# michiyasunaga/qagnn

Hardware: AMD Instinct MI355X
Metric: QA-subgraphs/sec (batch x num_choice) fwd+bwd (higher is better)
Workload: dtype f32; 1 GPU; configs[1]: CSQA-shaped batch 64 questions x 5 choices = 320 subgraphs per GPU, n=200 node slots, 400..2000 edges/subgraph, 38 relations (run_qagnn__csqa.sh), 5-layer GAT d=200 H=4, QAGNN decoder fwd+bwd (LM encoder excluded: random sent_vecs), dropout 0.2, train-mode BN; subgraphs_per_gpu=320, nodes=64000, edges=396800, edges_with_self_loops=460800, graph_input=load-time int32 blobs (qagnn_graph_from_blobs), 13.3 B/edge on the wire, parallelism=single

## Files before the change

### __graft_entry__.py

```python
import os
import sys

ROOT = os.path.dirname(os.path.abspath(__file__))
if ROOT not in sys.path:
    sys.path.insert(0, ROOT)


def build():
    from qagnn_amd.build import build as build_lib
    path = build_lib(force=False)
    from qagnn_amd import _lib
    lib = _lib.load_library(path)
    assert lib.qagnn_abi_version() == _lib.ABI_VERSION
    for name in _lib.EXPORTS + _lib.EXPORTS_TN + _lib.EXPORTS_INFER + _lib.EXPORTS_LOSS + _lib.EXPORTS_EXPLAIN + _lib.EXPORTS_DEFER:
        assert hasattr(lib, name), name
    import qagnn_amd.modeling_qagnn
    import oracle.qagnn_oracle
    print(f'[build] {path} ok ({os.path.getsize(path)} bytes), {len(_lib.EXPORTS)} C-ABI symbols')


def smoke():
    import torch
    sys.path.insert(0, os.path.join(ROOT, 'tests'))
    import helpers
    from qagnn_amd import modeling_qagnn as MQ
    from qagnn_amd import ops
    assert torch.cuda.is_available(), 'smoke() needs an MI355X'
    torch.set_num_threads(min(os.cpu_count() or 1, 32))
    case = dict(shape='config1', nq=1, nc=5, n=100, n_rel=17, std=0.6, train=True, seed=3,
# ... 32 lines not shown
```

### qagnn_amd/_lib.py

```python
import ctypes as C
import functools
import os

import torch

_HERE = os.path.dirname(os.path.abspath(__file__))
LIB_PATH = os.environ.get('QAGNN_LIB') or os.path.join(_HERE, 'libqagnn_hip.so')

EXPORTS = ['qagnn_last_error', 'qagnn_abi_version', 'qagnn_graph_storage_elems', 'qagnn_graph_prep', 'qagnn_graph_prep_blocked',
           'qagnn_graph_from_blobs', 'qagnn_radam_step_f32', 'qagnn_node_prep_f32', 'qagnn_seed_epoch_advance', 'qagnn_seed_epoch_set',
           'qagnn_gemm_nn_f32', 'qagnn_gemm_nn_split_f32', 'qagnn_gemm_nn_pack_bytes', 'qagnn_gemm_nn_ws_bytes', 'qagnn_gemm_nn_split_ws_f32', 'qagnn_gemm_nn_prepack_bytes', 'qagnn_gemm_nn_prepack_f32',
           'qagnn_gemm_nn_prepack_clear', 'qagnn_gemm_tn_workspace_elems', 'qagnn_gemm_tn_f32', 'qagnn_gemm_tn2_f32', 'qagnn_gemm_tn_colsum_f32',
           'qagnn_colreduce_workspace_elems', 'qagnn_colreduce_f32', 'qagnn_bn_finalize_f32', 'qagnn_bn_stats_finalize_f32', 'qagnn_bn_relu_bwd_f32',
           'qagnn_gelu_dropout_fwd_f32', 'qagnn_gelu_dropout_bwd_f32', 'qagnn_sin_basis_f32',
           'qagnn_bn_relu_bwd_colsum_f32',
           'qagnn_pool_attn_fwd_f32', 'qagnn_pool_attn_bwd_f32', 'qagnn_head_post_fwd_f32', 'qagnn_head_post_bwd_f32', 'qagnn_add_row0_f32', 'qagnn_gather_multi_f32', 'qagnn_gather_multi_sum_f32',
           'qagnn_edge_attn_fwd_f32', 'qagnn_edge_attn_bwd_f32',
           'qagnn_hop_fwd_workspace_elems', 'qagnn_hop_bwd_workspace_elems', 'qagnn_hop_fwd_f32', 'qagnn_hop_bwd_f32',
           'qagnn_stack_fwd_f32', 'qagnn_stack_bwd_f32', 'qagnn_absmax_f32', 'qagnn_zero_words', 'qagnn_gemm_tn_h2_f32', 'qagnn_gelu_dropout_fwd_amax_f32', 'qagnn_gelu_dropout_amax_scratch_elems',
           'qagnn_timing_enable', 'qagnn_timing_read', 'qagnn_gemm_tn_h1_f32', 'qagnn_gelu_dropout_bwd_amax_f32', 'qagnn_packed_min_rows',
           'qagnn_radam_step_scaled_f32', 'qagnn_grad_norm_workspace_elems', 'qagnn_grad_norm_f32', 'qagnn_scale_multi_f32', 'qagnn_graph_prep_cap',
           'qagnn_store_gather', 'qagnn_graph_from_store']
EXPORTS_TN = ['qagnn_gemm_tn_graph_f32', 'qagnn_gemm_tn_route_query', 'qagnn_tn_work_table', 'qagnn_tn_live_tiles']
EXPORTS_INFER = ['qagnn_infer_version', 'qagnn_bn_relu_absmax_scratch_elems', 'qagnn_bn_relu_absmax_f32', 'qagnn_stack_infer_f32',
                 'qagnn_choice_eval_f32']
EXPORTS_LOSS = ['qagnn_loss_version', 'qagnn_choice_loss_f32', 'qagnn_choice_loss_bwd_f32']
EXPORTS_EXPLAIN = ['qagnn_explain_version', 'qagnn_attn_export_f32', 'qagnn_attn_trace_f32']
EXPORTS_DEFER = ['qagnn_defer_version', 'qagnn_stack_bwd_defer_elems', 'qagnn_stack_bwd_deferred_f32']
EXPORTS_ROWS = ['qagnn_rows_version', 'qagnn_row_groups_workspace_elems', 'qagnn_row_groups', 'qagnn_row_segment_sum_workspace_elems',
                'qagnn_row_segment_sum_f32', 'qagnn_rows_scatter_f32']
ROWS_CHUNK = 64
ROWS_MAX_N, ROWS_MAX_TABLE = 1 << 20, 1 << 26
DEFER_MAX_HOPS = 16
TRACE_MAX_N = 1024
LOSS_KINDS = {'cross_entropy': 0, 'margin_rank': 1}
LOSS_THREADS = 256

CLS_SLICES = 4
ABI_VERSION = 25

_i32, _i64, _f32, _u64, _vp = C.c_int32, C.c_int64, C.c_float, C.c_uint64, C.c_void_p


class qagnn_graph(C.Structure):
    _fields_ = ([(n, _i32) for n in ('N', 'E', 'Ep', 'R', 'T', 'C')] +
# ... 144 lines not shown
    lib.qagnn_explain_version.argtypes = []
    lib.qagnn_attn_export_f32.argtypes = [C.POINTER(qagnn_graph), _vp, _i64, _i32, _vp, _i64, _vp]
    lib.qagnn_attn_trace_f32.argtypes = [C.POINTER(qagnn_graph), _vp, _i64, _i32, _i32, _i32, _i32, _i32, _vp, _vp, _vp, _vp]
    lib.qagnn_defer_version.argtypes = []
    lib.qagnn_stack_bwd_defer_elems.restype = _i64
    lib.qagnn_stack_bwd_defer_elems.argtypes = [_i32, _i32, _i32, _i32]
    lib.qagnn_stack_bwd_deferred_f32.argtypes = [C.POINTER(qagnn_hop_args), _i32, _vp, _i64, _vp]
    lib.qagnn_rows_version.argtypes = []
    lib.qagnn_row_groups_workspace_elems.restype = _i64
    lib.qagnn_row_groups_workspace_elems.argtypes = [_i32]
    lib.qagnn_row_groups.argtypes = [_vp, _i32, _i64, _vp, _vp, _vp, _vp, _vp, _i64, _vp]
    lib.qagnn_row_segment_sum_workspace_elems.restype = _i64
    lib.qagnn_row_segment_sum_workspace_elems.argtypes = [_i32, _i32]
    lib.qagnn_row_segment_sum_f32.argtypes = [_vp, _i64, _i32, _vp, _vp, _vp, _i32, _vp, _i64, _i32, _vp, _i64, _vp]
    lib.qagnn_rows_scatter_f32.argtypes = [_vp, _i64, _i32, _vp, _vp, _i32, _vp, _i64, _i64, _i32, _vp]
    for name in EXPORTS + EXPORTS_TN + EXPORTS_INFER + EXPORTS_LOSS + EXPORTS_EXPLAIN + EXPORTS_DEFER + EXPORTS_ROWS:
        fn = getattr(lib, name)
        if fn.restype is C.c_int and name not in ('qagnn_abi_version',):
            fn.restype = _i32
    return lib


def _ptr(t):
    return None if t is None else t.data_ptr()


def choice_loss_bound(kind, nc, Q, max_abs=1.0, margin=0.0, weight=1.0, threads=LOSS_THREADS):
    import math
    u, v = 2.0 ** -24, 2.0 ** -53
    M, L, w = max(1.0, float(max_abs)), math.log(nc), abs(float(weight))
    S = -(-Q // threads) + math.log2(threads) + nc
    if LOSS_KINDS[kind] == 0:
        return w * M * (u * (nc + 8 + 5 * L) + v * S * (2 + L)), w / Q * u * (nc + 8 + L)
    return w * M * (3 * u + v * S) * (2 + abs(float(margin)) / M), w / Q * 2 * u


def _running_fields(running):
    if running is None:
        return None, None, None, None, 0, 0.0, 1.0
# ... 502 lines not shown
        return out

    def gemm_tn_graph(self, A1, A2, B, graph=None, pieces=3, amax=None, out=None):
        _chkp(A1, 'A1'), _chkp(A2, 'A2'), _chkp(B, 'B')
        Ka1, Ka2 = A1.size(1), A2.size(1)
        R, No = B.shape
        assert A1.size(0) == R and A2.size(0) == R and (pieces == 3 or amax is not None)
        out, ws = self._tn_out_ws(R, Ka1 + Ka2, No, out, B.device)
        am = [None, None, None] if amax is None else [t.data_ptr() for t in amax]
        rc = self.lib.qagnn_gemm_tn_graph_f32(A1.data_ptr(), _ld(A1), Ka1, A2.data_ptr(), _ld(A2), Ka2, B.data_ptr(), _ld(B), out.data_ptr(), _ld(out),
                                              R, No, am[0], am[1], am[2], pieces, C.byref(graph.c) if graph is not None else None, ws.data_ptr(),
                                              self._stream())
        self._check(rc, 'qagnn_gemm_tn_graph_f32')
        return out

    def tn_route_query(self, R, Ka1, Ka2, No):
        out = (_i32 * 4)()
        self._check(self.lib.qagnn_gemm_tn_route_query(R, Ka1, Ka2, No, C.cast(out, _vp)), 'qagnn_gemm_tn_route_query')
        return tuple(out)

    def tn_work_table(self, graph, S, chunk_tiles):
        out = torch.empty(4 + 5 * S, dtype=torch.int32, device=graph.storage.device)
        self._check(self.lib.qagnn_tn_work_table(C.byref(graph.c), S, chunk_tiles, out.data_ptr(), self._stream()), 'qagnn_tn_work_table')
        return out

    def tn_live_tiles(self, on):
        return int(self.lib.qagnn_tn_live_tiles(int(on)))

    def gemm_tn2(self, A1, A2, B, out=None):
        _chkp(A1, 'A1'), _chkp(A2, 'A2'), _chkp(B, 'B')
# ... 617 lines not shown
```

### qagnn_amd/build.py

```python
import hashlib
import os
import subprocess
import sys

HERE = os.path.dirname(os.path.abspath(__file__))
CSRC = os.path.join(HERE, 'csrc')
LIB = os.path.join(HERE, 'libqagnn_hip.so')
STAMP = LIB + '.srchash'
SOURCES = ['graph_prep.hip', 'gemm.hip', 'elementwise.hip', 'edge_attn.hip', 'pool.hip', 'hop.hip', 'optim.hip', 'gemm_split.hip', 'gemm_nn2.hip', 'gemm_dispatch.hip', 'timing.hip', 'infer.hip', 'loss.hip', 'explain.hip', 'rows.hip']
FLAGS = ['--offload-arch=gfx950', '-O3', '-std=c++17', '-fPIC', '-shared']


def hashed_files():
    headers = sorted(f for f in os.listdir(CSRC) if f.endswith('.h'))
    return [os.path.join(CSRC, s) for s in SOURCES + headers] + [os.path.join(HERE, '..', 'include', 'qagnn_hip.h'),
                                                                 os.path.join(HERE, '..', 'include', 'qagnn_hip_tn.h'),
                                                                 os.path.join(HERE, '..', 'include', 'qagnn_hip_infer.h'),
                                                                 os.path.join(HERE, '..', 'include', 'qagnn_hip_loss.h'),
                                                                 os.path.join(HERE, '..', 'include', 'qagnn_hip_explain.h'),
                                                                 os.path.join(HERE, '..', 'include', 'qagnn_hip_defer.h'),
                                                                 os.path.join(HERE, '..', 'include', 'qagnn_hip_rows.h')]


def source_hash():
    h = hashlib.sha256(' '.join(FLAGS).encode())
    for p in hashed_files():
        with open(p, 'rb') as f:
            h.update(os.path.basename(p).encode() + b'\0' + f.read() + b'\0')
    return h.hexdigest()


def up_to_date():
    if not (os.path.exists(LIB) and os.path.exists(STAMP)):
        return False
    with open(STAMP) as f:
        return f.read().strip() == source_hash()
# ... 20 lines not shown
```

### qagnn_amd/csrc/common.h

```cpp
#pragma once
#include <hip/hip_runtime.h>
#include <stdint.h>
#include <stdio.h>

#include <type_traits>

#include "../../include/qagnn_hip.h"
#include "../../include/qagnn_hip_tn.h"
#include "../../include/qagnn_hip_infer.h"

namespace qagnn {

void set_error(const char* fmt, ...);

struct NnProduct {
  const qagnn_gemm_nn_args* a;
  bool split;
  const float* B1n; int ldn1; const float* B2n; int ldn2;
  void* ws; int64_t ws_bytes;
};
enum class NnFamily { FP32, SPLIT, NN2 };
enum class NnB { IN_KERNEL, PACK, IMAGE };
struct NnRoute {
  NnFamily family;
// ... 7 lines not shown
  static int n = [] {
    int dev = 0, v = 0;
    if (hipGetDevice(&dev) != hipSuccess || hipDeviceGetAttribute(&v, hipDeviceAttributeMultiprocessorCount, dev) != hipSuccess || v <= 0) v = 256;
    return v;
  }();
  return n;
}
static inline int cdiv(int64_t a, int64_t b) { return (int)((a + b - 1) / b); }
inline void nn_grid(NnRoute& r, int M, int No, int rows_per_tile, int per_cu) {
  r.ntiles = cdiv(No, r.nt * 16) * cdiv(M, rows_per_tile);
  const int cap = (num_cus() * per_cu) & ~7;
  r.grid = r.ntiles < cap ? r.ntiles : cap;
}
NnRoute nn_route(const NnProduct& p);
bool nn_rows_packed(int64_t M);
int gemm_nn(const NnProduct& p, hipStream_t stream);
int launch_nn(const NnRoute& r, const qagnn_gemm_nn_args& a, hipStream_t stream);
int launch_nn_split(const NnRoute& r, const qagnn_gemm_nn_args& a, const float* B1n, int ldn1, const float* B2n, int ldn2, hipStream_t stream);
int launch_nn2(const NnRoute& r, const qagnn_gemm_nn_args& a, const float* B1n, int ldn1, const float* B2n, int ldn2, hipStream_t stream);
int launch_pack_b(int np, const qagnn_gemm_nn_args& a, const float* B1n, int ldn1, const float* B2n, int ldn2, void* ws, hipStream_t stream);
namespace nn2 { int walk_tiles(int K1, int K2); }
int64_t nn2_pack_bytes(int No, int K1, int K2, int np);
const void* nn2_prepack_lookup(const float* B1n, int ldn1, int K1, const float* B2n, int ldn2, int K2, int No, int np);

struct TnProduct {
  const float* A1; int lda1, Ka1;
  const float* A2; int lda2, Ka2; bool two;
  const float* B; int ldb;
  float* C; int ldc, R, No;
  const float* a_scale; const float* a_shift; const int64_t* a_rowidx; int accumulate;
  float* bsum; const int64_t* b_rowidx; int groups;
  const uint32_t* amax[3]; int np;
  float* ws;
  const qagnn_graph* g;
};
// ... 309 lines not shown
```

### qagnn_amd/csrc/gemm_dispatch.hip

```cpp
#include <stdlib.h>

#include <atomic>
#include <initializer_list>

#include "common.h"

namespace qagnn {

static int pick_nt(int No) {
  const int cands[5] = {13, 7, 8, 4, 2};
  for (int c : cands)
    if (No % (c * 16) == 0) return c;
  int best = 4;
  int64_t best_cost = INT64_MAX;
  for (int c : cands) {
    const int64_t cost = (int64_t)cdiv(No, c * 16) * c * 16;
    if (cost < best_cost) { best_cost = cost; best = c; }
  }
  return best;
}

static std::atomic<int64_t> g_pack_min_m{8192};
bool nn_rows_packed(int64_t M) { return M >= g_pack_min_m.load(std::memory_order_relaxed); }

static bool nn2_ok(const qagnn_gemm_nn_args& a, int ldn1, int ldn2) {
  const int64_t lim = (int64_t)0x7FFFFFFF;
  if (a.a_rowidx && !(a.a_rows > 0 && a.a_rows * (int64_t)a.lda1 * 4 < lim && a.K2 == 0)) return false;
  if (a.K1 % 8 != 0 || a.K2 % 8 != 0) return false;
  if ((int64_t)a.M * a.lda1 * 4 >= lim || (int64_t)a.No * ldn1 * 4 >= lim || (int64_t)a.M * a.ldc * 4 >= lim) return false;
  if (a.K2 > 0 && ((int64_t)a.M * a.lda2 * 4 >= lim || (int64_t)a.No * ldn2 * 4 >= lim)) return false;
  if (a.K2 > 0 && (a.K1 & 31) != 0 && a.K2 < 32 - (a.K1 & 31)) return false;
  if (a.a_scale && a.K1 > 256) return false;
  return true;
}
static bool nn2_staggered(int nt, const qagnn_gemm_nn_args& a) {
  return nt >= 8 && nn2::walk_tiles(a.K1, a.K2) >= 10 && (int64_t)cdiv(a.No, nt * 16) * cdiv(a.M, 256) * 10 >= num_cus() * 9;
}

NnRoute nn_route(const NnProduct& p) {
  const qagnn_gemm_nn_args& a = *p.a;
  NnRoute r = {};
  r.np = 3;
  r.affine = a.a_scale != nullptr;
  if (!p.split) {
    r.family = NnFamily::FP32;
    r.nt = pick_nt(a.No);
    r.wv = 8;
    nn_grid(r, a.M, a.No, 128, QAGNN_NN_OCC > 0 ? QAGNN_NN_OCC : 1);
    return r;
  }
  const int nt16 = cdiv(a.No, 16);
  r.nt = nt16 >= 13 ? 13 : nt16 >= 8 ? 8 : nt16 >= 7 ? 7 : nt16 >= 4 ? 4 : 2;
  for (int c : {7, 4, 2})
    if (cdiv(a.M, 128) * cdiv(a.No, r.nt * 16) < num_cus() * 3 / 2 && c < r.nt) r.nt = c;
  r.wv = 4;
  r.stats = a.colstat_part != nullptr;
  if (!nn2_ok(a, p.ldn1, p.ldn2)) {
    const int64_t lim = (int64_t)0x7FFFFFFF;
    r.family = NnFamily::SPLIT;
    r.flat = a.a_rowidx || (int64_t)a.M * a.lda1 * 4 >= lim || (int64_t)a.M * a.lda2 * 4 >= lim || (int64_t)a.No * p.ldn1 * 4 >= lim ||
             (int64_t)a.No * p.ldn2 * 4 >= lim;
    nn_grid(r, a.M, a.No, 128, 2);
    return r;
  }
  r.family = NnFamily::NN2;
  auto image = [&](int np) {
    const int64_t need = nn2_pack_bytes(a.No, a.K1, a.K2, np);
    if ((r.image = nn2_prepack_lookup(p.B1n, p.ldn1, a.K1, p.B2n, p.ldn2, a.K2, a.No, np))) r.b = NnB::IMAGE;
    else if (p.ws && nn_rows_packed(a.M) && p.ws_bytes >= need && (np == 3 || aligned16(p.ws))) { r.b = NnB::PACK; r.ws_bytes = need; }
    else return false;
    r.np = np;
    return true;
  };
  const bool scaled = nn_rows_packed(a.M) && a.a_amax1 && (a.K2 == 0 || a.a_amax2);
  if (!(scaled && image(a.pieces == 1 ? 1 : 2)) && !image(3)) r.b = NnB::IN_KERNEL;
  if (r.b != NnB::IN_KERNEL && r.np == 3 && nn2_staggered(r.nt, a)) r.wv = 8;
  nn_grid(r, a.M, a.No, r.wv * 32, r.wv == 8 ? 1 : 2);
  return r;
}

static int nn_validate(const NnProduct& p) {
  QAGNN_REQUIRE(p.a, QAGNN_EINVAL, "gemm_nn: null pointer");
  const qagnn_gemm_nn_args& a = *p.a;
  const float* B1 = p.split ? p.B1n : a.B1, *B2 = p.split ? p.B2n : a.B2;
  const int ldb1 = p.split ? p.ldn1 : a.ldb1, ldb2 = p.split ? p.ldn2 : a.ldb2, km = p.split ? 4 : 16;
  QAGNN_REQUIRE(a.A1 && B1 && a.C, QAGNN_EINVAL, "gemm_nn: null pointer");
  QAGNN_REQUIRE(a.M > 0 && a.No > 0 && a.K1 > 0, QAGNN_EINVAL, "gemm_nn: bad sizes M=%d No=%d K1=%d", a.M, a.No, a.K1);
  QAGNN_REQUIRE(a.K1 % km == 0 && a.K2 % km == 0 && a.K2 >= 0, QAGNN_EINVAL, "gemm_nn: K1=%d K2=%d must be multiples of %d", a.K1, a.K2, km);
  QAGNN_REQUIRE(a.No % 4 == 0, QAGNN_EINVAL, "gemm_nn: No=%d must be a multiple of 4", a.No);
  QAGNN_REQUIRE(a.lda1 % 4 == 0 && ldb1 % 4 == 0 && (!p.split || ldb1 >= a.K1) && aligned16(a.A1) && aligned16(B1), QAGNN_EINVAL,
                "gemm_nn: operand 1 must be 16-byte aligned with pitches multiple of 4");
  QAGNN_REQUIRE(a.K2 == 0 || (a.A2 && B2 && a.lda2 % 4 == 0 && ldb2 % 4 == 0 && (!p.split || ldb2 >= a.K2) && aligned16(a.A2) && aligned16(B2)),
                QAGNN_EINVAL, "gemm_nn: operand 2 must be 16-byte aligned with pitches multiple of 4");
  QAGNN_REQUIRE(!a.rowtab || a.rowidx, QAGNN_EINVAL, "gemm_nn: rowtab without rowidx");
  QAGNN_REQUIRE(a.ldc % 4 == 0 && aligned16(a.C) && (!a.bias || aligned16(a.bias)) && (!a.rowtab || (aligned16(a.rowtab) && a.ldt % 4 == 0)),
                QAGNN_EINVAL, "gemm_nn: C / bias / rowtab must be 16-byte aligned with pitches multiple of 4");
// ... 14 lines not shown
}

int gemm_nn(const NnProduct& p, hipStream_t stream) {
  TimedScope timed(0, stream);
  if (int rc = nn_validate(p)) return rc;
  const qagnn_gemm_nn_args& a = *p.a;
  const NnRoute r = nn_route(p);
  if (r.family == NnFamily::FP32) return launch_nn(r, a, stream);
  if (r.family == NnFamily::SPLIT) return launch_nn_split(r, a, p.B1n, p.ldn1, p.B2n, p.ldn2, stream);
  if (r.b == NnB::IN_KERNEL) return launch_nn2(r, a, p.B1n, p.ldn1, p.B2n, p.ldn2, stream);
  if (r.b == NnB::PACK) {
    QAGNN_REQUIRE(aligned16(p.ws), QAGNN_EINVAL, "gemm_nn: the pack workspace must be 16-byte aligned");
    if (int rc = launch_pack_b(r.np, a, p.B1n, p.ldn1, p.B2n, p.ldn2, p.ws, stream)) return rc;
  }
  return launch_nn2(r, a, static_cast<const float*>(r.b == NnB::PACK ? p.ws : r.image), cdiv(a.No, 16), nullptr, 0, stream);
}

static int tn_chunk_rows(int R, int blocks_per_chunk, int per_cu, int ktile, int lo) {
  const int target = num_cus() * per_cu / blocks_per_chunk;
  const int rows = cdiv(cdiv(R, target > 0 ? target : 1), ktile) * ktile, lo_k = cdiv(lo, ktile) * ktile;
  return rows > lo_k ? rows : lo_k;
}
static int tn_min_chunk(int R, bool split) { return R > 4096 ? 256 : split ? 32 : 64; }
static int64_t tn_ws_bound(int R, int Ka, int No) { return (int64_t)cdiv(R, tn_min_chunk(R, true)) * ((int64_t)Ka * No + 4 * (int64_t)No); }
constexpr int TN_WS_MIN_TILES = 28;

static int pick_tn_waves(int Ka) {
  int best = 4, best_waste = INT32_MAX;
  for (int nw = 16; nw >= 4; --nw) {
    const int bm = nw * 16, waste = cdiv(Ka, bm) * bm - Ka;
// ... 121 lines not shown

extern "C" int qagnn_gemm_nn_f32(const qagnn_gemm_nn_args* a, qagnn_stream_t stream) {
  return gemm_nn(NnProduct{a, false, nullptr, 0, nullptr, 0, nullptr, 0}, (hipStream_t)stream);
}

extern "C" int qagnn_gemm_nn_split_f32(const qagnn_gemm_nn_args* a, const float* B1n, int32_t ldn1, const float* B2n, int32_t ldn2,
                                       qagnn_stream_t stream) {
  return gemm_nn(NnProduct{a, true, B1n, ldn1, B2n, ldn2, nullptr, 0}, (hipStream_t)stream);
}

extern "C" int qagnn_gemm_nn_split_ws_f32(const qagnn_gemm_nn_args* a, const float* B1n, int32_t ldn1, const float* B2n, int32_t ldn2,
                                          void* ws, int64_t ws_bytes, qagnn_stream_t stream) {
  return gemm_nn(NnProduct{a, true, B1n, ldn1, B2n, ldn2, ws, ws_bytes}, (hipStream_t)stream);
}

extern "C" int64_t qagnn_gemm_tn_workspace_elems(int32_t R, int32_t Ka, int32_t No) { return tn_ws_bound(R, Ka, No); }

extern "C" int qagnn_gemm_tn_colsum_f32(const float* A, int32_t lda, const float* B, int32_t ldb, float* C, int32_t ldc, int32_t R,
                                        int32_t Ka, int32_t No, const float* a_scale, const float* a_shift, const int64_t* a_rowidx,
                                        int32_t accumulate, float* bsum, const int64_t* b_rowidx, int32_t groups, float* workspace,
                                        qagnn_stream_t stream) {
  TnProduct p = tn_product(A, lda, Ka, nullptr, 0, 0, B, ldb, C, ldc, R, No, a_scale, a_shift, workspace);
  p.a_rowidx = a_rowidx; p.accumulate = accumulate; p.bsum = bsum; p.b_rowidx = b_rowidx; p.groups = groups;
  return gemm_tn(p, (hipStream_t)stream);
}

extern "C" int qagnn_gemm_tn_f32(const float* A, int32_t lda, const float* B, int32_t ldb, float* C, int32_t ldc, int32_t R,
                                 int32_t Ka, int32_t No, const float* a_scale, const float* a_shift, const int64_t* a_rowidx,
                                 int32_t accumulate, float* workspace, qagnn_stream_t stream) {
  TnProduct p = tn_product(A, lda, Ka, nullptr, 0, 0, B, ldb, C, ldc, R, No, a_scale, a_shift, workspace);
// ... 53 lines not shown
```

### qagnn_amd/csrc/gemm_nn2.hip

```cpp
#include <stdlib.h>


#include "gemm_device.h"

namespace qagnn {

namespace nn2 {

constexpr int BK = 32;

template <bool AFFINE, int NP = 2>
__device__ __forceinline__ void split_frag2(const u32x4s (&r)[2], u32x4s (&f)[NP], const float* __restrict__ sc, const float* __restrict__ sh, float lo,
                                            float s) {
  uint32_t ph[4], pl[4];
#pragma unroll
  for (int e = 0; e < 8; e += 2) {
    const uint32_t ux = r[e >> 2][e & 3], uy = r[(e + 1) >> 2][(e + 1) & 3];
    float x = __builtin_bit_cast(float, ux), y = __builtin_bit_cast(float, uy);
    if constexpr (AFFINE) {
      x = floor_nan(fmaf(x, sc[e], sh[e]), lo);
      y = floor_nan(fmaf(y, sc[e + 1], sh[e + 1]), lo);
    }
    if constexpr (NP == 2) split2(x, y, s, ph[e >> 1], pl[e >> 1]);
    else split1(x, y, s, ph[e >> 1]);
// ... 446 lines not shown
      __syncthreads();
      QAGNN_NN_SLAB_FILL(acc[i], (lane >> 4) * 4)
      __syncthreads();
      if constexpr (STATS) {
        const float* const S0 = reinterpret_cast<const float*>(smem) + (w & ~3) * SLAB_ROWS * PS;
        QAGNN_NN_SLAB_STATS(S0, i == 0, M - (m0 + (w * 2 + i) * 16), No)
      }
      QAGNN_NN_SLAB_STORE(m0 + (w * 2 + i) * 16, M, No)
    }
    if constexpr (STATS) QAGNN_NN_STATS_PUT(true, WV / 4, M, No)
  }
}
#undef QAGNN_NN2_SIX
#undef QAGNN_NN2_SIX_T

template <int NT, bool AFFINE, bool STATS, int NP, bool PACKED, int WV>
static int launch_i(const NnRoute& r, const qagnn_gemm_nn_args& b, const float* B1n, int ldn1, const float* B2n, int ldn2, hipStream_t stream) {
  const size_t lds = nn2_lds_bytes<NT, STATS, WV, NP>(AFFINE ? 2 * ((b.K1 + 31) & ~31) * 4 : 0);
  constexpr int lds_max = nn2_lds_bytes<NT, STATS, WV, NP>(AFFINE ? 2 * 256 * 4 : 0);
  if (int rc = raise_lds_limit<k_gemm_nn2<NT, AFFINE, STATS, NP, PACKED, WV>>(lds_max, "k_gemm_nn2")) return rc;
  k_gemm_nn2<NT, AFFINE, STATS, NP, PACKED, WV><<<r.grid, WV * 64, lds, stream>>>(b, B1n, ldn1, B2n, ldn2, r.ntiles);
  QAGNN_LAUNCH_CHECK("k_gemm_nn2");
  return QAGNN_OK;
}

template <int NP>
__device__ __forceinline__ void pack_b_wave(const float* __restrict__ B1n, int ldn1, int K1, const float* __restrict__ B2n, int ldn2, int K2, int No,
                                            int NJ, int nkt, int it, int j, unsigned char* __restrict__ out) {
  const int lane = threadIdx.x & 63;
  if (j >= NJ) return;
// ... 86 lines not shown
  return dispatch_int<13, 8, 7, 4, 2>(r.nt, [&](auto nt) {
    return dispatch_int<0, 1, 2, 3, 4>(shape, [&](auto sh) {
      constexpr int NT = nt.value, NP = (sh.value == 0 || sh.value == 4) ? 3 : sh.value, WV = sh.value == 4 ? 8 : 4;
      constexpr bool PACKED = sh.value != 0;
      if constexpr (WV == 8 && NT != 13 && NT != 8) {
        set_error("k_gemm_nn2: no staggered block with %d column tiles", NT);
        return QAGNN_EUNSUPPORTED;
      } else {
        if constexpr (NT != 8) {
          if (r.stats) return nn2::launch_i<NT, false, true, NP, PACKED, WV>(r, b, B1n, ldn1, B2n, ldn2, stream);
        }
        return dispatch_bool(r.affine, [&](auto aff) { return nn2::launch_i<NT, aff.value, false, NP, PACKED, WV>(r, b, B1n, ldn1, B2n, ldn2, stream); });
      }
    });
  });
}

int64_t nn2_pack_bytes(int No, int K1, int K2, int np) {
  const int64_t img = ((int64_t)nn2::walk_tiles(K1, K2) * cdiv(No, 16) + 13) * (np * 1024);
  return np <= 2 ? img + (((int64_t)cdiv(No, 16) + 13) * 4 + 15) / 16 * 16 : img;
}

int launch_pack_b(int np, const qagnn_gemm_nn_args& a, const float* B1n, int ldn1, const float* B2n, int ldn2, void* ws, hipStream_t stream) {
  const int NJ = cdiv(a.No, 16), nkt = nn2::walk_tiles(a.K1, a.K2);
  return dispatch_int<3, 2, 1>(np, [&](auto p) {
    nn2::k_pack_b<p.value><<<dim3(cdiv(NJ, 4), nkt), 256, 0, stream>>>(B1n, ldn1, a.K1, B2n, ldn2, a.K2, a.No, NJ, nkt, reinterpret_cast<unsigned char*>(ws));
    QAGNN_LAUNCH_CHECK("k_pack_b");
    return QAGNN_OK;
  });
}
// ... 81 lines not shown
```

### qagnn_amd/csrc/hop.hip

```cpp
#include "common.h"
#include "../../include/qagnn_hip_defer.h"

#include <mutex>

namespace qagnn {

static inline int64_t up4(int64_t x) { return (x + 3) & ~(int64_t)3; }
static inline int64_t max64(int64_t a, int64_t b) { return a > b ? a : b; }

static inline int hop_stat_tiles(int N) { return cdiv(N, 128); }
static inline bool hop_stat_width(int DP) { return DP > 192 && DP <= 208; }
static int64_t hop_pack_elems(int DP) { return up4((qagnn_gemm_nn_pack_bytes(3 * DP, DP, DP) + 3) / 4); }
static inline int hop_cls_part_rows(const qagnn_graph* g) { return QAGNN_CLS_SLICES * g->C + g->max_chunks; }

struct HopWs {
  float* base;
  int64_t total = 0;
  float* take(int64_t n) { const int64_t o = total; total += up4(n); return base ? base + o : nullptr; }
};
struct HopFwdWs : HopWs {
  const int64_t N, Ep, DP, ampart_elems = max64(N, gelu_amax_scratch_elems(N * DP));
  float* const score = take(Ep * 4);
  float* const crws = take(max64(qagnn_colreduce_workspace_elems(N, DP, 1), hop_stat_tiles(N) * 3 * DP));
  float* const pkws = take(hop_pack_elems(DP));
// ... 275 lines not shown
    QAGNN_REQUIRE(h->tab_col + h->T <= SP, QAGNN_EINVAL, "hop_bwd: tab_col=%d + T=%d exceeds SP=%d", h->tab_col, h->T, SP);
    if (h->dTT != h->dWs_t + (int64_t)h->tab_col * 3 * DP) {
      hipError_t he = hipMemcpyAsync(h->dTT, h->dWs_t + (int64_t)h->tab_col * 3 * DP, (size_t)h->T * 3 * DP * sizeof(float), hipMemcpyDeviceToDevice,
                                     (hipStream_t)wstream);
      if (he != hipSuccess) { set_error("hop_bwd: dTT copy failed: %s", hipGetErrorString(he)); return QAGNN_EHIP; }
    }
  } else {
    HOP_TRY(qagnn_colreduce_f32(0, dKMQ, 3 * DP, nullptr, 3 * DP, N, 3 * DP, h->ntype, h->T, nullptr, nullptr, nullptr, nullptr, nullptr, 1.0f, h->dTT,
                                w.crws, stream));
  }
  if (ss->side) {
    *done = ss->take();
    hipError_t he = hipEventRecord(*done, ss->side);
    QAGNN_REQUIRE(he == hipSuccess, QAGNN_EHIP, "hop_bwd: hipEventRecord failed: %s", hipGetErrorString(he));
  }
  if (h->dX) {
    qagnn_gemm_nn_args gx = {};
    gx.A1 = dKMQ; gx.lda1 = 3 * DP; gx.K1 = 3 * DP; gx.B1 = h->Wx; gx.ldb1 = DP; gx.C = h->dX; gx.ldc = DP; gx.M = N; gx.No = DP;
    gx.accumulate = h->accumulate_dX;
    nn_scaled(h, &gx, w_dkmq);
    HOP_TRY(hop_nn(h, &gx, h->Wx_t, 3 * DP, nullptr, 0, w.pkws, stream));
  }
  if (SP > 0 && h->dS) {
    qagnn_gemm_nn_args gs = {};
    gs.A1 = dKMQ; gs.lda1 = 3 * DP; gs.K1 = 3 * DP; gs.B1 = h->Ws; gs.ldb1 = SP; gs.C = h->dS; gs.ldc = SP; gs.M = N; gs.No = SP;
    gs.accumulate = h->accumulate_dS;
    nn_scaled(h, &gs, w_dkmq);
    HOP_TRY(hop_nn(h, &gs, h->Ws_t, 3 * DP, nullptr, 0, w.pkws, stream));
  }
  return QAGNN_OK;
}

static_assert(QAGNN_HOP_AM_DH1 == QAGNN_HOP_AM_DOUT + 1 && QAGNN_HOP_AM_DKMQ == QAGNN_HOP_AM_DOUT + 2, "the backward's words are three in a row");
__global__ void k_zero_bwd_words(uint32_t* __restrict__ amax, int k) {
  for (int i = threadIdx.x; i < 3 * k; i += blockDim.x) amax[(i / 3) * QAGNN_HOP_AMAX_WORDS + QAGNN_HOP_AM_DOUT + i % 3] = 0u;
}
static int zero_bwd_words(const qagnn_hop_args* hops, int k, hipStream_t main) {
  bool all = true, any = false, one_array = true;
  for (int l = 0; l < k; ++l) {
    const bool h2 = hop_amax_stack(hops, k, l).on && hop_stat_width(hops[l].DP);
    all = all && h2;
    any = any || h2;
    one_array = one_array && hops[l].amax != nullptr && hops[l].amax == hops[0].amax + (int64_t)l * QAGNN_HOP_AMAX_WORDS;
  }
// ... 125 lines not shown
```

Baseline: 46500 QA-subgraphs/s.

## Fuse hop backward dX and dS GEMMs into one dual-output kernel

Adds a dual-output NN GEMM kernel that reads the shared dKMQ operand once and computes both dX (No=200) and dS (No≈112) products in a single launch. Both packed weight images sit in LDS together. The hop backward uses this path when the pair qualifies and falls back to two separate GEMMs otherwise. This is meant to halve A-operand traffic and remove one launch per hop, at the cost of larger LDS use and higher register pressure per block, which lowers occupancy.

```diff
diff --git a/__graft_entry__.py b/__graft_entry__.py
--- a/__graft_entry__.py
+++ b/__graft_entry__.py
@@ -12,7 +12,7 @@
     from qagnn_amd import _lib
     lib = _lib.load_library(path)
     assert lib.qagnn_abi_version() == _lib.ABI_VERSION
-    for name in _lib.EXPORTS + _lib.EXPORTS_TN + _lib.EXPORTS_INFER + _lib.EXPORTS_LOSS + _lib.EXPORTS_EXPLAIN + _lib.EXPORTS_DEFER:
+    for name in _lib.EXPORTS + _lib.EXPORTS_TN + _lib.EXPORTS_INFER + _lib.EXPORTS_LOSS + _lib.EXPORTS_EXPLAIN + _lib.EXPORTS_DEFER + _lib.EXPORTS_ROWS + _lib.EXPORTS_DUAL:
         assert hasattr(lib, name), name
     import qagnn_amd.modeling_qagnn
     import oracle.qagnn_oracle
diff --git a/include/qagnn_hip_dual.h b/include/qagnn_hip_dual.h
--- /dev/null
+++ b/include/qagnn_hip_dual.h
@@ -0,0 +1,28 @@
+#ifndef QAGNN_HIP_DUAL_H
+#define QAGNN_HIP_DUAL_H
+
+#include "qagnn_hip.h"
+
+#ifdef __cplusplus
+extern "C" {
+#endif
+
+int qagnn_dual_version(void);
+
+int qagnn_gemm_nn_dual_f32(const qagnn_gemm_nn_args* p1, const float* B1n, int32_t ldn1, const qagnn_gemm_nn_args* p2, const float* B2n,
+                           int32_t ldn2, void* pack_ws, int64_t pack_bytes, qagnn_stream_t stream);
+
+int qagnn_gemm_nn_dual_query(const qagnn_gemm_nn_args* p1, const float* B1n, int32_t ldn1, const qagnn_gemm_nn_args* p2, const float* B2n,
+                             int32_t ldn2, const void* pack_ws, int64_t pack_bytes);
+
+int64_t qagnn_dual_launches(void);
+
+int qagnn_dual_blocks_per_cu(void);
+
+int qagnn_nn_dual_enable(int32_t on);
+
+#ifdef __cplusplus
+}
+#endif
+
+#endif
diff --git a/qagnn_amd/_lib.py b/qagnn_amd/_lib.py
--- a/qagnn_amd/_lib.py
+++ b/qagnn_amd/_lib.py
@@ -29,6 +29,8 @@
 EXPORTS_DEFER = ['qagnn_defer_version', 'qagnn_stack_bwd_defer_elems', 'qagnn_stack_bwd_deferred_f32']
 EXPORTS_ROWS = ['qagnn_rows_version', 'qagnn_row_groups_workspace_elems', 'qagnn_row_groups', 'qagnn_row_segment_sum_workspace_elems',
                 'qagnn_row_segment_sum_f32', 'qagnn_rows_scatter_f32']
+EXPORTS_DUAL = ['qagnn_dual_version', 'qagnn_gemm_nn_dual_f32', 'qagnn_gemm_nn_dual_query', 'qagnn_dual_launches', 'qagnn_dual_blocks_per_cu',
+                'qagnn_nn_dual_enable']
 ROWS_CHUNK = 64
 ROWS_MAX_N, ROWS_MAX_TABLE = 1 << 20, 1 << 26
 DEFER_MAX_HOPS = 16
@@ -203,7 +205,14 @@
     lib.qagnn_row_segment_sum_workspace_elems.argtypes = [_i32, _i32]
     lib.qagnn_row_segment_sum_f32.argtypes = [_vp, _i64, _i32, _vp, _vp, _vp, _i32, _vp, _i64, _i32, _vp, _i64, _vp]
     lib.qagnn_rows_scatter_f32.argtypes = [_vp, _i64, _i32, _vp, _vp, _i32, _vp, _i64, _i64, _i32, _vp]
-    for name in EXPORTS + EXPORTS_TN + EXPORTS_INFER + EXPORTS_LOSS + EXPORTS_EXPLAIN + EXPORTS_DEFER + EXPORTS_ROWS:
+    lib.qagnn_dual_version.argtypes = []
+    lib.qagnn_gemm_nn_dual_f32.argtypes = [C.POINTER(qagnn_gemm_nn_args), _vp, _i32, C.POINTER(qagnn_gemm_nn_args), _vp, _i32, _vp, _i64, _vp]
+    lib.qagnn_gemm_nn_dual_query.argtypes = [C.POINTER(qagnn_gemm_nn_args), _vp, _i32, C.POINTER(qagnn_gemm_nn_args), _vp, _i32, _vp, _i64]
+    lib.qagnn_dual_launches.restype = _i64
+    lib.qagnn_dual_launches.argtypes = []
+    lib.qagnn_nn_dual_enable.argtypes = [_i32]
+    lib.qagnn_dual_blocks_per_cu.argtypes = []
+    for name in EXPORTS + EXPORTS_TN + EXPORTS_INFER + EXPORTS_LOSS + EXPORTS_EXPLAIN + EXPORTS_DEFER + EXPORTS_ROWS + EXPORTS_DUAL:
         fn = getattr(lib, name)
         if fn.restype is C.c_int and name not in ('qagnn_abi_version',):
             fn.restype = _i32
@@ -212,6 +221,15 @@
 
 def _ptr(t):
     return None if t is None else t.data_ptr()
+
+
+def dual_args(A, lda, M, K, a_amax, C1, ldc1, No1, C2, ldc2, No2, accumulate1=False, accumulate2=False):
+    out = []
+    for Cp, ldc, No, acc in ((C1, ldc1, No1, accumulate1), (C2, ldc2, No2, accumulate2)):
+        a = qagnn_gemm_nn_args()
+        a.A1, a.lda1, a.K1, a.C, a.ldc, a.M, a.No, a.accumulate, a.a_amax1 = A, lda, K, Cp, ldc, M, No, 1 if acc else 0, a_amax
+        out.append(a)
+    return out
 
 
 def choice_loss_bound(kind, nc, Q, max_abs=1.0, margin=0.0, weight=1.0, threads=LOSS_THREADS):
@@ -744,6 +762,24 @@
         self._check(rc, 'qagnn_gemm_tn_graph_f32')
         return out
 
+    def gemm_nn_dual(self, A, B1n, B2n, a_amax, out1, out2, accumulate1=False, accumulate2=False, ws=None):
+        for t, n in ((A, 'A'), (B1n, 'B1n'), (B2n, 'B2n'), (out1, 'out1'), (out2, 'out2')):
+            _chkp(t, n)
+        assert ws is None or (ws.is_cuda and ws.dtype == torch.uint8 and ws.is_contiguous())
+        a1, a2 = dual_args(A.data_ptr(), _ld(A), A.size(0), A.size(1), _ptr(a_amax), out1.data_ptr(), _ld(out1), B1n.size(0),
+                           out2.data_ptr(), _ld(out2), B2n.size(0), accumulate1, accumulate2)
+        rc = self.lib.qagnn_gemm_nn_dual_f32(C.byref(a1), B1n.data_ptr(), _ld(B1n), C.byref(a2), B2n.data_ptr(), _ld(B2n),
+                                             _ptr(ws), ws.numel() if ws is not None else 0, self._stream())
+        if rc != 2:
+            self._check(rc, 'qagnn_gemm_nn_dual_f32')
+        return rc
+
+    def nn_dual_enable(self, on):
+        return int(self.lib.qagnn_nn_dual_enable(int(on)))
+
+    def dual_launches(self):
+        return int(self.lib.qagnn_dual_launches())
+
     def tn_route_query(self, R, Ka1, Ka2, No):
         out = (_i32 * 4)()
         self._check(self.lib.qagnn_gemm_tn_route_query(R, Ka1, Ka2, No, C.cast(out, _vp)), 'qagnn_gemm_tn_route_query')
diff --git a/qagnn_amd/build.py b/qagnn_amd/build.py
--- a/qagnn_amd/build.py
+++ b/qagnn_amd/build.py
@@ -19,7 +19,8 @@
                                                                  os.path.join(HERE, '..', 'include', 'qagnn_hip_loss.h'),
                                                                  os.path.join(HERE, '..', 'include', 'qagnn_hip_explain.h'),
                                                                  os.path.join(HERE, '..', 'include', 'qagnn_hip_defer.h'),
-                                                                 os.path.join(HERE, '..', 'include', 'qagnn_hip_rows.h')]
+                                                                 os.path.join(HERE, '..', 'include', 'qagnn_hip_rows.h'),
+                                                                 os.path.join(HERE, '..', 'include', 'qagnn_hip_dual.h')]
 
 
 def source_hash():
diff --git a/qagnn_amd/csrc/common.h b/qagnn_amd/csrc/common.h
--- a/qagnn_amd/csrc/common.h
+++ b/qagnn_amd/csrc/common.h
@@ -45,11 +45,24 @@
 }
 NnRoute nn_route(const NnProduct& p);
 bool nn_rows_packed(int64_t M);
+int nn_validate(const NnProduct& p);
 int gemm_nn(const NnProduct& p, hipStream_t stream);
 int launch_nn(const NnRoute& r, const qagnn_gemm_nn_args& a, hipStream_t stream);
 int launch_nn_split(const NnRoute& r, const qagnn_gemm_nn_args& a, const float* B1n, int ldn1, const float* B2n, int ldn2, hipStream_t stream);
 int launch_nn2(const NnRoute& r, const qagnn_gemm_nn_args& a, const float* B1n, int ldn1, const float* B2n, int ldn2, hipStream_t stream);
 int launch_pack_b(int np, const qagnn_gemm_nn_args& a, const float* B1n, int ldn1, const float* B2n, int ldn2, void* ws, hipStream_t stream);
+struct NnDual {
+  const float* A; int lda, K, M;
+  const uint32_t* a_amax;
+  const void* image[2];
+  float* C[2]; int ldc[2], No[2], accumulate[2];
+};
+int launch_nn2_dual(const NnDual& d, hipStream_t stream);
+int nn2_dual_blocks_per_cu();
+struct NnDualRoute { bool ok; NnDual d; bool pack[2]; int64_t ws_off[2]; };
+NnDualRoute nn_dual_route(const NnProduct& p1, const NnProduct& p2);
+int gemm_nn_dual(const NnProduct& p1, const NnProduct& p2, const NnDualRoute& r, hipStream_t stream);
+bool nn_dual_enabled();
 namespace nn2 { int walk_tiles(int K1, int K2); }
 int64_t nn2_pack_bytes(int No, int K1, int K2, int np);
 const void* nn2_prepack_lookup(const float* B1n, int ldn1, int K1, const float* B2n, int ldn2, int K2, int No, int np);
diff --git a/qagnn_amd/csrc/gemm_dispatch.hip b/qagnn_amd/csrc/gemm_dispatch.hip
--- a/qagnn_amd/csrc/gemm_dispatch.hip
+++ b/qagnn_amd/csrc/gemm_dispatch.hip
@@ -4,6 +4,7 @@
 #include <initializer_list>
 
 #include "common.h"
+#include "../../include/qagnn_hip_dual.h"
 
 namespace qagnn {
 
@@ -36,6 +37,8 @@
 static bool nn2_staggered(int nt, const qagnn_gemm_nn_args& a) {
   return nt >= 8 && nn2::walk_tiles(a.K1, a.K2) >= 10 && (int64_t)cdiv(a.No, nt * 16) * cdiv(a.M, 256) * 10 >= num_cus() * 9;
 }
+
+static bool nn_few_blocks(int M, int No, int nt) { return cdiv(M, 128) * cdiv(No, nt * 16) < num_cus() * 3 / 2; }
 
 NnRoute nn_route(const NnProduct& p) {
   const qagnn_gemm_nn_args& a = *p.a;
@@ -52,7 +55,7 @@
   const int nt16 = cdiv(a.No, 16);
   r.nt = nt16 >= 13 ? 13 : nt16 >= 8 ? 8 : nt16 >= 7 ? 7 : nt16 >= 4 ? 4 : 2;
   for (int c : {7, 4, 2})
-    if (cdiv(a.M, 128) * cdiv(a.No, r.nt * 16) < num_cus() * 3 / 2 && c < r.nt) r.nt = c;
+    if (nn_few_blocks(a.M, a.No, r.nt) && c < r.nt) r.nt = c;
   r.wv = 4;
   r.stats = a.colstat_part != nullptr;
   if (!nn2_ok(a, p.ldn1, p.ldn2)) {
@@ -79,7 +82,7 @@
   return r;
 }
 
-static int nn_validate(const NnProduct& p) {
+int nn_validate(const NnProduct& p) {
   QAGNN_REQUIRE(p.a, QAGNN_EINVAL, "gemm_nn: null pointer");
   const qagnn_gemm_nn_args& a = *p.a;
   const float* B1 = p.split ? p.B1n : a.B1, *B2 = p.split ? p.B2n : a.B2;
@@ -124,6 +127,58 @@
     if (int rc = launch_pack_b(r.np, a, p.B1n, p.ldn1, p.B2n, p.ldn2, p.ws, stream)) return rc;
   }
   return launch_nn2(r, a, static_cast<const float*>(r.b == NnB::PACK ? p.ws : r.image), cdiv(a.No, 16), nullptr, 0, stream);
+}
+
+static std::atomic<int> g_nn_dual{-1};
+static std::atomic<int64_t> g_nn_dual_launches{0};
+static int nn_dual_mode() {
+  static const int env = [] { const char* e = getenv("QAGNN_NN_DUAL"); const int v = e ? atoi(e) : 1; return v < 0 ? 0 : (v > 2 ? 2 : v); }();
+  const int v = g_nn_dual.load(std::memory_order_relaxed);
+  return v < 0 ? env : v;
+}
+bool nn_dual_enabled() { return nn_dual_mode() != 0; }
+
+NnDualRoute nn_dual_route(const NnProduct& p1, const NnProduct& p2) {
+  NnDualRoute r = {};
+  if (!p1.split || !p2.split) return r;
+  const qagnn_gemm_nn_args& a = *p1.a, &b = *p2.a;
+  if (a.A1 != b.A1 || a.lda1 != b.lda1 || a.K1 != b.K1 || a.M != b.M || a.a_amax1 != b.a_amax1 || !a.a_amax1) return r;
+  if (a.pieces == 1 || b.pieces == 1) return r;
+  for (const qagnn_gemm_nn_args* q : {&a, &b})
+    if (q->K2 != 0 || q->bias || q->rowtab || q->a_scale || q->a_shift || q->colstat_part || q->a_rowidx) return r;
+  if (cdiv(a.No, 16) != 13 || cdiv(b.No, 16) != 7) return r;
+  if (!nn2_ok(a, p1.ldn1, 0) || !nn2_ok(b, p2.ldn1, 0) || !nn_rows_packed(a.M)) return r;
+  if (nn_dual_mode() != 2 && (nn_few_blocks(a.M, a.No, 13) || nn_few_blocks(b.M, b.No, 7))) return r;
+  const NnProduct* ps[2] = {&p1, &p2};
+  int64_t used = 0;
+  for (int i = 0; i < 2; ++i) {
+    const qagnn_gemm_nn_args& q = *ps[i]->a;
+    r.d.image[i] = nn2_prepack_lookup(ps[i]->B1n, ps[i]->ldn1, q.K1, nullptr, 0, 0, q.No, 2);
+    if (!r.d.image[i]) {
+      const int64_t need = (nn2_pack_bytes(q.No, q.K1, 0, 2) + 15) & ~(int64_t)15;
+      if (!p1.ws || !aligned16(p1.ws) || used + need > p1.ws_bytes) return r;
+      r.pack[i] = true;
+      r.ws_off[i] = used;
+      r.d.image[i] = static_cast<const unsigned char*>(p1.ws) + used;
+      used += need;
+    }
+  }
+  r.d.A = a.A1; r.d.lda = a.lda1; r.d.K = a.K1; r.d.M = a.M; r.d.a_amax = a.a_amax1;
+  r.d.C[0] = a.C; r.d.ldc[0] = a.ldc; r.d.No[0] = a.No; r.d.accumulate[0] = a.accumulate;
+  r.d.C[1] = b.C; r.d.ldc[1] = b.ldc; r.d.No[1] = b.No; r.d.accumulate[1] = b.accumulate;
+  r.ok = true;
+  return r;
+}
+
+int gemm_nn_dual(const NnProduct& p1, const NnProduct& p2, const NnDualRoute& r, hipStream_t stream) {
+  TimedScope timed(0, stream);
+  const NnProduct* ps[2] = {&p1, &p2};
+  for (int i = 0; i < 2; ++i)
+    if (r.pack[i])
+      if (int rc = launch_pack_b(2, *ps[i]->a, ps[i]->B1n, ps[i]->ldn1, nullptr, 0, static_cast<unsigned char*>(p1.ws) + r.ws_off[i], stream)) return rc;
+  if (int rc = launch_nn2_dual(r.d, stream)) return rc;
+  g_nn_dual_launches.fetch_add(1, std::memory_order_relaxed);
+  return QAGNN_OK;
 }
 
 static int tn_chunk_rows(int R, int blocks_per_chunk, int per_cu, int ktile, int lo) {
@@ -275,6 +330,40 @@
   return gemm_nn(NnProduct{a, true, B1n, ldn1, B2n, ldn2, ws, ws_bytes}, (hipStream_t)stream);
 }
 
+extern "C" int qagnn_dual_version(void) { return 1; }
+
+extern "C" int qagnn_gemm_nn_dual_f32(const qagnn_gemm_nn_args* p1, const float* B1n, int32_t ldn1, const qagnn_gemm_nn_args* p2, const float* B2n,
+                                      int32_t ldn2, void* pack_ws, int64_t pack_bytes, qagnn_stream_t stream) {
+  const NnProduct q1{p1, true, B1n, ldn1, nullptr, 0, pack_ws, pack_bytes}, q2{p2, true, B2n, ldn2, nullptr, 0, nullptr, 0};
+  QAGNN_REQUIRE(p1 && p2, QAGNN_EINVAL, "gemm_nn_dual: null pointer");
+  QAGNN_REQUIRE(p1->K2 == 0 && p2->K2 == 0, QAGNN_EUNSUPPORTED, "gemm_nn_dual: one K segment per product (K2 = %d / %d)", p1->K2, p2->K2);
+  if (int rc = nn_validate(q1)) return rc;
+  if (int rc = nn_validate(q2)) return rc;
+  const NnDualRoute r = nn_dual_route(q1, q2);
+  QAGNN_REQUIRE(r.ok, QAGNN_EUNSUPPORTED, "gemm_nn_dual: not a pair the two-output launch takes (include/qagnn_hip_dual.h)");
+  return gemm_nn_dual(q1, q2, r, (hipStream_t)stream);
+}
+
+extern "C" int qagnn_gemm_nn_dual_query(const qagnn_gemm_nn_args* p1, const float* B1n, int32_t ldn1, const qagnn_gemm_nn_args* p2, const float* B2n,
+                                        int32_t ldn2, const void* pack_ws, int64_t pack_bytes) {
+  alignas(16) static char any_ws;
+  const bool assume = !pack_ws && pack_bytes < 0;
+  const NnProduct q1{p1, true, B1n, ldn1, nullptr, 0, assume ? &any_ws : const_cast<void*>(pack_ws), assume ? INT64_MAX : pack_bytes};
+  const NnProduct q2{p2, true, B2n, ldn2, nullptr, 0, nullptr, 0};
+  if (nn_validate(q1) != QAGNN_OK || nn_validate(q2) != QAGNN_OK) return 0;
+  return nn_dual_route(q1, q2).ok ? 1 : 0;
+}
+
+extern "C" int64_t qagnn_dual_launches(void) { return g_nn_dual_launches.load(); }
+
+extern "C" int qagnn_dual_blocks_per_cu(void) { return nn2_dual_blocks_per_cu(); }
+
+extern "C" int qagnn_nn_dual_enable(int32_t on) {
+  const int was = nn_dual_mode();
+  if (on >= 0) g_nn_dual.store(on > 2 ? 2 : on);
+  return was;
+}
+
 extern "C" int64_t qagnn_gemm_tn_workspace_elems(int32_t R, int32_t Ka, int32_t No) { return tn_ws_bound(R, Ka, No); }
 
 extern "C" int qagnn_gemm_tn_colsum_f32(const float* A, int32_t lda, const float* B, int32_t ldb, float* C, int32_t ldc, int32_t R,
diff --git a/qagnn_amd/csrc/gemm_nn2.hip b/qagnn_amd/csrc/gemm_nn2.hip
--- a/qagnn_amd/csrc/gemm_nn2.hip
+++ b/qagnn_amd/csrc/gemm_nn2.hip
@@ -484,6 +484,174 @@
 #undef QAGNN_NN2_SIX
 #undef QAGNN_NN2_SIX_T
 
+template <int J0, int NTH, int NT>
+__device__ __forceinline__ void dual_add_old(f32x4s (&acc)[2][NT], const __amdgpu_buffer_rsrc_t rC, const uint32_t (&cv)[2], const uint32_t (&cl)[2]) {
+#pragma unroll
+  for (int i = 0; i < 2; ++i) {
+    f32x4s t[NTH];
+#pragma unroll
+    for (int j = 0; j < NTH; ++j) t[j] = bload<f32x4s>(rC, j + 1 < NTH ? cv[i] : cl[i], (uint32_t)j * 64u);
+#pragma unroll
+    for (int j = 0; j < NTH; ++j) acc[i][J0 + j] += t[j];
+  }
+}
+template <int J0, int NTH, int NT>
+__device__ __forceinline__ void dual_store(const f32x4s (&acc)[2][NT], const __amdgpu_buffer_rsrc_t rC, const uint32_t (&cv)[2], const uint32_t (&cl)[2]) {
+#pragma unroll
+  for (int i = 0; i < 2; ++i)
+#pragma unroll
+    for (int j = 0; j < NTH; ++j)
+      __builtin_amdgcn_raw_buffer_store_b128(__builtin_bit_cast(u32x4s, acc[i][J0 + j]), rC, (int)(j + 1 < NTH ? cv[i] : cl[i]), j * 64, 0);
+}
+
+template <int NT1, int NT2, int NP>
+__global__ __launch_bounds__(256) __attribute__((amdgpu_waves_per_eu(2, 2))) void k_gemm_nn2_dual(NnDual a, int ntiles) {
+  static_assert(NP == 2, "the three-MFMA form");
+  constexpr int NT = NT1 + NT2, BM = 128;
+  constexpr int IMG = NT * NP * 1024;
+  static_assert((NT * NP) % 4 == 0, "the DMA blocks of a k-tile are dealt out evenly over the four waves");
+  extern __shared__ __attribute__((aligned(16))) unsigned char smem[];
+
+  const int tid = threadIdx.x;
+  const int w = __builtin_amdgcn_readfirstlane(tid >> 6);
+  const int M = a.M, K = a.K;
+  const int nkt = (K + 31) >> 5;
+  const __amdgpu_buffer_rsrc_t rA = __builtin_amdgcn_make_buffer_rsrc(const_cast<float*>(a.A), 0, M * a.lda * 4, 0x00020000);
+  const __amdgpu_buffer_rsrc_t rC1 = __builtin_amdgcn_make_buffer_rsrc(a.C[0], 0, M * a.ldc[0] * 4, 0x00020000);
+  const __amdgpu_buffer_rsrc_t rC2 = __builtin_amdgcn_make_buffer_rsrc(a.C[1], 0, M * a.ldc[1] * 4, 0x00020000);
+  const unsigned char* const pk1 = static_cast<const unsigned char*>(a.image[0]);
+  const unsigned char* const pk2 = static_cast<const unsigned char*>(a.image[1]);
+  const uint32_t fa = __builtin_amdgcn_readfirstlane(h2_scale_field(a.a_amax[0]));
+  const float sa = h2_field_to_scale(fa);
+  uint32_t fb[NT];
+  {
+    const uint32_t* const bf1 = reinterpret_cast<const uint32_t*>(pk1 + ((int64_t)nkt * NT1 + 13) * (NP * 1024));
+    const uint32_t* const bf2 = reinterpret_cast<const uint32_t*>(pk2 + ((int64_t)nkt * NT2 + 13) * (NP * 1024));
+#pragma unroll
+    for (int j = 0; j < NT; ++j) fb[j] = __builtin_amdgcn_readfirstlane(j < NT1 ? bf1[j] : bf2[j - NT1]);
+  }
+
+  u32x4s ra[2][2];
+  for (int vb = blockIdx.x; vb < ntiles; vb += gridDim.x) {
+    const int m0 = xcd_remap(vb, ntiles) * BM;
+    uint32_t arow[2];
+    {
+      int t_ = tid;
+      asm volatile("" : "+v"(t_));
+#pragma unroll
+      for (int i = 0; i < 2; ++i) {
+        const int row = m0 + w * 32 + i * 16 + (t_ & 15);
+        arow[i] = row < M ? (uint32_t)row * (uint32_t)a.lda * 4u + (uint32_t)((t_ >> 4) & 3) * 32u : OOB;
+      }
+    }
+    f32x4s acc[2][NT];
+#pragma unroll
+    for (int i = 0; i < 2; ++i)
+#pragma unroll
+      for (int j = 0; j < NT; ++j) acc[i][j] = (f32x4s){0.f, 0.f, 0.f, 0.f};
+    u32x4s af[2][NP];
+
+#define QAGNN_DUAL_GLOAD(IT)                                                     \
+    {                                                                            \
+      const int kb_ = (IT)*32;                                                   \
+      int tg_ = tid;                                                             \
+      asm volatile("" : "+v"(tg_));                                              \
+      const bool ain_ = kb_ + ((tg_ >> 4) & 3) * 8 < K;                          \
+      _Pragma("unroll") for (int i = 0; i < 2; ++i) {                            \
+        const uint32_t off_ = ain_ ? arow[i] : OOB;                              \
+        ra[i][0] = bload<u32x4s>(rA, off_, (uint32_t)kb_ * 4u);                  \
+        ra[i][1] = bload<u32x4s>(rA, off_, (uint32_t)kb_ * 4u + 16u);            \
+      }                                                                          \
+    }
+#define QAGNN_DUAL_GLDS(IT, BUF)                                                                                         \
+    {                                                                                                                    \
+      const unsigned char* const s1_ = pk1 + (int64_t)(IT) * (NT1 * NP * 1024);                                          \
+      const unsigned char* const s2_ = pk2 + (int64_t)(IT) * (NT2 * NP * 1024);                                          \
+      int td_ = tid;                                                                                                     \
+      asm volatile("" : "+v"(td_));  \
+      const uint32_t vo_ = (uint32_t)(td_ & 63) * 16u;                                                                   \
+      _Pragma("unroll") for (int b = 0; b < NT * NP / 4; ++b) {                                                          \
+        const int blk_ = w + b * 4;                                                                                      \
+                                            \
+        const unsigned char* const src_ = blk_ < NT1 * NP ? s1_ + blk_ * 1024 : s2_ + (blk_ - NT1 * NP) * 1024;          \
+        __builtin_amdgcn_global_load_lds((const __attribute__((address_space(1))) void*)(src_ + vo_),                    \
+                                         (__attribute__((address_space(3))) void*)((BUF) + blk_ * 1024), 16, 0, 0);      \
+      }                                                                                                                  \
+    }
+#define QAGNN_DUAL_SPLIT_A                                                                                               \
+    {                                                                                                                    \
+      _Pragma("unroll") for (int i = 0; i < 2; ++i) split_frag2<false, NP>(ra[i], af[i], nullptr, nullptr, 0.f, sa);     \
+    }
+#define QAGNN_DUAL_MFMA_TILE(CUR)                                                                                        \
+    {                                                                                                                    \
+      __builtin_amdgcn_s_setprio(1);                                                                                     \
+      int tm_ = tid;                                                                                                     \
+      asm volatile("" : "+v"(tm_));                                                                                      \
+      const int rd_ = (((tm_ & 15) ^ (2 * ((tm_ >> 4) & 3))) + 16 * ((tm_ >> 4) & 3)) * 16;  \
+      u32x4s bfa[NP], bfb[NP];                                                                                           \
+      _Pragma("unroll") for (int p = 0; p < NP; ++p) bfa[p] = *reinterpret_cast<const u32x4s*>((CUR) + p * 1024 + rd_);  \
+      _Pragma("unroll") for (int j = 0; j < NT; ++j) {                                                                   \
+        u32x4s(&bf)[NP] = (j & 1) ? bfb : bfa;                                                                           \
+        u32x4s(&bn)[NP] = (j & 1) ? bfa : bfb;                                                                           \
+        if (j + 1 < NT) {                                                                                                \
+          _Pragma("unroll") for (int p = 0; p < NP; ++p)                                                                 \
+              bn[p] = *reinterpret_cast<const u32x4s*>((CUR) + ((j + 1) * NP + p) * 1024 + rd_);                         \
+        }                                                                                                                \
+        _Pragma("unroll") for (int i = 0; i < 2; ++i) acc[i][j] = mfma_pieces<NP, true>(af[i], bf, acc[i][j]);           \
+        __builtin_amdgcn_sched_barrier(0);                                                                               \
+      }                                                                                                                  \
+      __builtin_amdgcn_s_setprio(0);                                                                                     \
+    }
+
+    __syncthreads();
+    QAGNN_DUAL_GLOAD(0)
+    QAGNN_DUAL_GLDS(0, smem)
+    QAGNN_DUAL_SPLIT_A
+    __syncthreads();
+    for (int it = 0; it + 1 < nkt; ++it) {
+      unsigned char* const cur = smem + (it & 1) * IMG;
+      unsigned char* const nxt = smem + ((it & 1) ^ 1) * IMG;
+      QAGNN_DUAL_GLDS(it + 1, nxt)
+      QAGNN_DUAL_GLOAD(it + 1)
+      QAGNN_DUAL_MFMA_TILE(cur)
+      QAGNN_DUAL_SPLIT_A
+      __syncthreads();
+    }
+    {
+      unsigned char* const cur = smem + ((nkt - 1) & 1) * IMG;
+      QAGNN_DUAL_MFMA_TILE(cur)
+    }
+#undef QAGNN_DUAL_GLOAD
+#undef QAGNN_DUAL_GLDS
+#undef QAGNN_DUAL_SPLIT_A
+#undef QAGNN_DUAL_MFMA_TILE
+#pragma unroll
+    for (int j = 0; j < NT; ++j) {
+      uint32_t f = fb[j];
+      asm volatile("" : "+s"(f));
+      const float inv = h2_inv_scale(fa, f);
+#pragma unroll
+      for (int i = 0; i < 2; ++i) acc[i][j] *= inv;
+    }
+    int te = tid;
+    asm volatile("" : "+v"(te));
+    const int c4 = 4 * ((te >> 4) & 3), lrow = te & 15;
+    uint32_t cv1[2], cl1[2], cv2[2], cl2[2];
+#pragma unroll
+    for (int i = 0; i < 2; ++i) {
+      const int row = m0 + w * 32 + i * 16 + lrow;
+      cv1[i] = row < M ? (uint32_t)row * (uint32_t)a.ldc[0] * 4u + (uint32_t)c4 * 4u : OOB;
+      cv2[i] = row < M ? (uint32_t)row * (uint32_t)a.ldc[1] * 4u + (uint32_t)c4 * 4u : OOB;
+      cl1[i] = (NT1 - 1) * 16 + c4 < a.No[0] ? cv1[i] : OOB;
+      cl2[i] = (NT2 - 1) * 16 + c4 < a.No[1] ? cv2[i] : OOB;
+    }
+    if (a.accumulate[0]) dual_add_old<0, NT1>(acc, rC1, cv1, cl1);
+    if (a.accumulate[1]) dual_add_old<NT1, NT2>(acc, rC2, cv2, cl2);
+    dual_store<0, NT1>(acc, rC1, cv1, cl1);
+    dual_store<NT1, NT2>(acc, rC2, cv2, cl2);
+  }
+}
+
 template <int NT, bool AFFINE, bool STATS, int NP, bool PACKED, int WV>
 static int launch_i(const NnRoute& r, const qagnn_gemm_nn_args& b, const float* B1n, int ldn1, const float* B2n, int ldn2, hipStream_t stream) {
   const size_t lds = nn2_lds_bytes<NT, STATS, WV, NP>(AFFINE ? 2 * ((b.K1 + 31) & ~31) * 4 : 0);
@@ -600,6 +768,21 @@
       }
     });
   });
+}
+
+constexpr int NN2_DUAL_LDS = 2 * (13 + 7) * 2 * 1024;
+int launch_nn2_dual(const NnDual& d, hipStream_t stream) {
+  if (int rc = raise_lds_limit<nn2::k_gemm_nn2_dual<13, 7, 2>>(NN2_DUAL_LDS, "k_gemm_nn2_dual")) return rc;
+  const int ntiles = cdiv(d.M, 128), cap = (num_cus() * 2) & ~7;
+  nn2::k_gemm_nn2_dual<13, 7, 2><<<ntiles < cap ? ntiles : cap, 256, NN2_DUAL_LDS, stream>>>(d, ntiles);
+  QAGNN_LAUNCH_CHECK("k_gemm_nn2_dual");
+  return QAGNN_OK;
+}
+int nn2_dual_blocks_per_cu() {
+  int n = 0;
+  if (raise_lds_limit<nn2::k_gemm_nn2_dual<13, 7, 2>>(NN2_DUAL_LDS, "k_gemm_nn2_dual") != QAGNN_OK) return 0;
+  if (hipOccupancyMaxActiveBlocksPerMultiprocessor(&n, nn2::k_gemm_nn2_dual<13, 7, 2>, 256, NN2_DUAL_LDS) != hipSuccess) { (void)hipGetLastError(); return 0; }
+  return n;
 }
 
 int64_t nn2_pack_bytes(int No, int K1, int K2, int np) {
diff --git a/qagnn_amd/csrc/hop.hip b/qagnn_amd/csrc/hop.hip
--- a/qagnn_amd/csrc/hop.hip
+++ b/qagnn_amd/csrc/hop.hip
@@ -313,20 +313,26 @@
     hipError_t he = hipEventRecord(*done, ss->side);
     QAGNN_REQUIRE(he == hipSuccess, QAGNN_EHIP, "hop_bwd: hipEventRecord failed: %s", hipGetErrorString(he));
   }
+  qagnn_gemm_nn_args gx = {}, gs = {};
   if (h->dX) {
-    qagnn_gemm_nn_args gx = {};
     gx.A1 = dKMQ; gx.lda1 = 3 * DP; gx.K1 = 3 * DP; gx.B1 = h->Wx; gx.ldb1 = DP; gx.C = h->dX; gx.ldc = DP; gx.M = N; gx.No = DP;
     gx.accumulate = h->accumulate_dX;
     nn_scaled(h, &gx, w_dkmq);
-    HOP_TRY(hop_nn(h, &gx, h->Wx_t, 3 * DP, nullptr, 0, w.pkws, stream));
   }
   if (SP > 0 && h->dS) {
-    qagnn_gemm_nn_args gs = {};
     gs.A1 = dKMQ; gs.lda1 = 3 * DP; gs.K1 = 3 * DP; gs.B1 = h->Ws; gs.ldb1 = SP; gs.C = h->dS; gs.ldc = SP; gs.M = N; gs.No = SP;
     gs.accumulate = h->accumulate_dS;
     nn_scaled(h, &gs, w_dkmq);
-    HOP_TRY(hop_nn(h, &gs, h->Ws_t, 3 * DP, nullptr, 0, w.pkws, stream));
-  }
+  }
+  if (h->dX && SP > 0 && h->dS && h->gemm_split != 0 && nn_dual_enabled()) {
+    const NnProduct px{&gx, true, h->Wx_t, 3 * DP, nullptr, 0, w.pkws, hop_pack_elems(DP) * 4}, ps{&gs, true, h->Ws_t, 3 * DP, nullptr, 0, nullptr, 0};
+    HOP_TRY(nn_validate(px));
+    HOP_TRY(nn_validate(ps));
+    const NnDualRoute r = nn_dual_route(px, ps);
+    if (r.ok) return gemm_nn_dual(px, ps, r, (hipStream_t)stream);
+  }
+  if (h->dX) HOP_TRY(hop_nn(h, &gx, h->Wx_t, 3 * DP, nullptr, 0, w.pkws, stream));
+  if (SP > 0 && h->dS) HOP_TRY(hop_nn(h, &gs, h->Ws_t, 3 * DP, nullptr, 0, w.pkws, stream));
   return QAGNN_OK;
 }
 
```

Result: faster. 47020 QA-subgraphs/s, median of 6 (+1.1%).
